# HemuManju/carla-imitation-learning

Hardware: NVIDIA B200
Metric: bc_train_frames_per_sec (higher is better)
Workload: dtype bf16

## Files before the change

### carla_imitation_learning_b200/csrc/stage.cu

```cuda
#include "bc_common.cuh"

namespace {

__device__ __forceinline__ float gray_px(uint32_t r, uint32_t g, uint32_t b) {
    const float s = (float)(299u * r + 587u * g + 114u * b);
    const float rcp = 1.0f / 255000.0f;
    const float q0 = __fmul_rn(s, rcp);
    const float rem = __fmaf_rn(-q0, 255000.0f, s);
    return __fmaf_rn(rem, rcp, q0);
}

template <int PX, typename TOUT>
__global__ void __launch_bounds__(256) stage_gray_kernel(const uint8_t* __restrict__ rgb,
                                                         TOUT* __restrict__ out, int64_t n_groups) {
    const int64_t stride = (int64_t)gridDim.x * blockDim.x;
    for (int64_t g = (int64_t)blockIdx.x * blockDim.x + threadIdx.x; g < n_groups; g += stride) {
        const uint32_t* src = reinterpret_cast<const uint32_t*>(rgb + g * (3 * PX));
        uint32_t w[3 * PX / 4];
#pragma unroll
        for (int i = 0; i < 3 * PX / 4; ++i) w[i] = __ldg(src + i);
        float v[PX];
#pragma unroll
        for (int p = 0; p < PX; ++p) {
            uint32_t c[3];
#pragma unroll
            for (int k = 0; k < 3; ++k) {
                const int byte = 3 * p + k;
                c[k] = (w[byte >> 2] >> (8 * (byte & 3))) & 0xffu;
            }
            v[p] = gray_px(c[0], c[1], c[2]);
        }
        if constexpr (sizeof(TOUT) == 4) {
            float4* dst = reinterpret_cast<float4*>(out + g * PX);
#pragma unroll
            for (int i = 0; i < PX / 4; ++i) dst[i] = make_float4(v[4 * i], v[4 * i + 1], v[4 * i + 2], v[4 * i + 3]);
        } else {
            uint32_t pk[PX / 2];
#pragma unroll
            for (int i = 0; i < PX / 2; ++i) {
                __nv_bfloat162 h = __floats2bfloat162_rn(v[2 * i], v[2 * i + 1]);
                pk[i] = *reinterpret_cast<uint32_t*>(&h);
            }
            uint4* dst = reinterpret_cast<uint4*>(out + g * PX);
#pragma unroll
            for (int i = 0; i < PX / 8; ++i) dst[i] = make_uint4(pk[4 * i], pk[4 * i + 1], pk[4 * i + 2], pk[4 * i + 3]);
        }
    }
}

constexpr int TP_NG = 21, TP_NQ = 86;

template <typename LOADER>
__device__ __forceinline__ void tp_write(LOADER&& load16, __nv_bfloat16* __restrict__ out, int64_t u) {
    const int g = (int)(u % TP_NG), q = (int)((u / TP_NG) % TP_NQ), c = (int)((u / (TP_NG * TP_NQ)) % 3);
    const int64_t plane = u / (TP_NG * TP_NQ * 3);
    const int R = 3 * q + c;
    uint32_t pk[8] = {0, 0, 0, 0, 0, 0, 0, 0};
    if (R < BC_H) load16(plane, R, 12 * g, pk);
    __nv_bfloat16* dst = out + plane * BC_TP_PLANE_ELEMS + ((int64_t)(c * 2) * TP_NQ + q) * (TP_NG * 8) + g * 8;
    *reinterpret_cast<uint4*>(dst) = make_uint4(pk[0], pk[1], pk[2], pk[3]);
    *reinterpret_cast<uint4*>(dst + TP_NQ * TP_NG * 8) = make_uint4(pk[4], pk[5], pk[6], pk[7]);
}

__device__ __forceinline__ uint32_t pack_bf16(float a, float b) {
    __nv_bfloat162 h = __floats2bfloat162_rn(a, b);
    return *reinterpret_cast<uint32_t*>(&h);
}

constexpr int TP_NU = TP_NG + 1;

__device__ __forceinline__ float gray_px_bf16_exact(uint32_t px ) {
    uint32_t acc = __dp4a(px, 0xFF72FFFFu, 0x4B000000u);
    acc = __dp4a(px, 0x00004D2Cu, acc);
    const float s = __uint_as_float(acc) - 8388608.0f;
    constexpr float r = 1.0f / 255000.0f;
    constexpr float r_lo = (float)(1.0 / 255000.0 - (double)r);
    return __fmaf_rn(s, r_lo, __fmul_rn(s, r));
}

__global__ void __launch_bounds__(256) stage_gray_tp_kernel(const uint8_t* __restrict__ rgb, __nv_bfloat16* __restrict__ out,
                                                            __nv_bfloat16* __restrict__ plain, uint32_t n_units) {
    bc::pdl_wait();
    bc::pdl_trigger();
    const uint32_t stride = gridDim.x * blockDim.x;
    for (uint32_t u = blockIdx.x * blockDim.x + threadIdx.x; u < n_units; u += stride) {
        const uint32_t t1 = u / TP_NU, g = u - t1 * TP_NU;
        const uint32_t t2 = t1 / TP_NQ, q = t1 - t2 * TP_NQ;
        const uint32_t plane = t2 / 3u, c = t2 - plane * 3u;
        const uint32_t R = 3u * q + c;
        uint32_t pk[6] = {0, 0, 0, 0, 0, 0};
        if (R < BC_H) {
            const uint32_t* src = reinterpret_cast<const uint32_t*>(rgb + ((size_t)plane * (BC_H * BC_W) + R * BC_W + 12u * g) * 3);
            uint32_t w[10];
#pragma unroll
            for (int i = 0; i < 9; ++i) w[i] = (g < TP_NG || i < 3) ? __ldg(src + i) : 0u;
            w[9] = 0u;
            float v[12];
#pragma unroll
            for (int p = 0; p < 12; ++p) {
                constexpr uint32_t sel[4] = {0x1210u, 0x2321u, 0x3432u, 0x4543u};
                const int o = (3 * p) & 3, i = (3 * p) >> 2;
                v[p] = gray_px_bf16_exact(__byte_perm(w[i], w[i + 1], sel[o]));
            }
#pragma unroll
            for (int i = 0; i < 6; ++i) pk[i] = pack_bf16(v[2 * i], v[2 * i + 1]);
            if (plain) {
                uint2* dst = reinterpret_cast<uint2*>(plain + ((size_t)plane * BC_H + R) * BC_W + 12u * g);
                dst[0] = make_uint2(pk[0], pk[1]);
                if (g < TP_NG) { dst[1] = make_uint2(pk[2], pk[3]); dst[2] = make_uint2(pk[4], pk[5]); }
            }
        }
        __nv_bfloat16* row0 = out + (size_t)plane * BC_TP_PLANE_ELEMS + ((c * 2u) * TP_NQ + q) * (TP_NG * 8);
        __nv_bfloat16* row1 = row0 + TP_NQ * TP_NG * 8;
        if (g < TP_NG) {
            *reinterpret_cast<uint4*>(row0 + g * 8) = make_uint4(pk[0], pk[1], pk[2], pk[3]);
            *reinterpret_cast<uint2*>(row1 + g * 8) = make_uint2(pk[4], pk[5]);
        }
        if (g > 0) *reinterpret_cast<uint2*>(row1 + (g - 1) * 8 + 4) = make_uint2(pk[0], pk[1]);
    }
}

template <typename TIN>
__global__ void __launch_bounds__(256) planes_to_tp_kernel(const TIN* __restrict__ in, int64_t plane_stride, __nv_bfloat16* __restrict__ out, int64_t n_units) {
    const int64_t stride = (int64_t)gridDim.x * blockDim.x;
    for (int64_t u = (int64_t)blockIdx.x * blockDim.x + threadIdx.x; u < n_units; u += stride)
        tp_write([&](int64_t plane, int R, int px0, uint32_t (&pk)[8]) {
            const TIN* src = in + plane * plane_stride + R * BC_W + px0;
            if constexpr (sizeof(TIN) == 4) {
#pragma unroll
                for (int i = 0; i < 4; ++i) {
                    const float4 f = __ldg(reinterpret_cast<const float4*>(src) + i);
                    pk[2 * i] = pack_bf16(f.x, f.y); pk[2 * i + 1] = pack_bf16(f.z, f.w);
                }
            } else {
#pragma unroll
                for (int i = 0; i < 4; ++i) {
                    const uint2 w = __ldg(reinterpret_cast<const uint2*>(src) + i);
                    pk[2 * i] = w.x; pk[2 * i + 1] = w.y;
                }
            }
        }, out, u);
}

struct AugRow { float cy, cx, br, ct, sa, mean, istd, pad; };
__device__ __forceinline__ float clamp255(float v) { return fminf(fmaxf(v, 0.f), 255.f); }
__device__ __forceinline__ float luma(float r, float g, float b) {
    return __fadd_rn(__fadd_rn(__fmul_rn(0.299f, r), __fmul_rn(0.587f, g)), __fmul_rn(0.114f, b));
}
__device__ __forceinline__ float aug_px(const uint8_t* __restrict__ px, const AugRow& t) {
    float c[3];
#pragma unroll
    for (int k = 0; k < 3; ++k) {
        float v = clamp255(__fmul_rn((float)__ldg(px + k), t.br));
        c[k] = clamp255(__fadd_rn(__fmul_rn(__fadd_rn(v, -127.5f), t.ct), 127.5f));
    }
    const float y = luma(c[0], c[1], c[2]);
#pragma unroll
    for (int k = 0; k < 3; ++k) c[k] = clamp255(__fadd_rn(y, __fmul_rn(__fadd_rn(c[k], -y), t.sa)));
    const float g = __fmul_rn(luma(c[0], c[1], c[2]), 1.0f / 255.0f);
    return __fmul_rn(__fadd_rn(g, -t.mean), t.istd);
}

__global__ void __launch_bounds__(256) stage_aug_f32_kernel(const uint8_t* __restrict__ rgb, int src_h, int src_w, const AugRow* __restrict__ table,
                                                            float* __restrict__ out, int64_t n_groups) {
    const int64_t stride = (int64_t)gridDim.x * blockDim.x;
    for (int64_t u = (int64_t)blockIdx.x * blockDim.x + threadIdx.x; u < n_groups; u += stride) {
        const int x4 = (int)(u % (BC_W / 4)), R = (int)((u / (BC_W / 4)) % BC_H);
        const int64_t plane = u / ((BC_W / 4) * BC_H);
        const AugRow t = table[plane];
        const uint8_t* src = rgb + ((plane * src_h + (int)t.cy + R) * (int64_t)src_w + (int)t.cx + 4 * x4) * 3;
        float4 v;
        v.x = aug_px(src, t); v.y = aug_px(src + 3, t); v.z = aug_px(src + 6, t); v.w = aug_px(src + 9, t);
        reinterpret_cast<float4*>(out)[u] = v;
    }
}

__global__ void __launch_bounds__(256) stage_aug_tp_kernel(const uint8_t* __restrict__ rgb, int src_h, int src_w, const AugRow* __restrict__ table,
                                                           __nv_bfloat16* __restrict__ out, int64_t n_units) {
    const int64_t stride = (int64_t)gridDim.x * blockDim.x;
    for (int64_t u = (int64_t)blockIdx.x * blockDim.x + threadIdx.x; u < n_units; u += stride) {
        const int g = (int)(u % TP_NU), q = (int)((u / TP_NU) % TP_NQ), c = (int)((u / (TP_NU * TP_NQ)) % 3);
        const int64_t plane = u / (TP_NU * TP_NQ * 3);
        const int R = 3 * q + c;
        uint32_t pk[6] = {0, 0, 0, 0, 0, 0};
        if (R < BC_H) {
            const AugRow t = table[plane];
            const uint8_t* src = rgb + ((plane * src_h + (int)t.cy + R) * (int64_t)src_w + (int)t.cx + 12 * g) * 3;
            const int npx = g < TP_NG ? 12 : 4;
            float v[12];
#pragma unroll
            for (int p = 0; p < 12; ++p) v[p] = p < npx ? aug_px(src + 3 * p, t) : 0.f;
#pragma unroll
            for (int i = 0; i < 6; ++i) pk[i] = pack_bf16(v[2 * i], v[2 * i + 1]);
        }
        __nv_bfloat16* row0 = out + plane * BC_TP_PLANE_ELEMS + ((int64_t)(c * 2) * TP_NQ + q) * (TP_NG * 8);
        __nv_bfloat16* row1 = row0 + TP_NQ * TP_NG * 8;
        if (g < TP_NG) {
            *reinterpret_cast<uint4*>(row0 + g * 8) = make_uint4(pk[0], pk[1], pk[2], pk[3]);
            *reinterpret_cast<uint2*>(row1 + g * 8) = make_uint2(pk[4], pk[5]);
        }
        if (g > 0) *reinterpret_cast<uint2*>(row1 + (g - 1) * 8 + 4) = make_uint2(pk[0], pk[1]);
    }
}

}

extern "C" int bc_stage_augment(const uint8_t* rgb, int64_t n_frames, int src_h, int src_w, const float* table, void* out, int out_dtype, void* stream) {
    BC_CHECK_ARG(rgb && table && out && n_frames >= 0, "bc_stage_augment: null pointer");
    BC_CHECK_ARG(src_h >= BC_H && src_w >= BC_W, "bc_stage_augment: source frames %dx%d are smaller than the %dx%d crop", src_h, src_w, BC_H, BC_W);
    BC_CHECK_ARG(out_dtype == BC_F32 || out_dtype == BC_BF16_TP, "bc_stage_augment: output is BC_F32 planes or BC_BF16_TP planes, got %d", out_dtype);
    BC_CHECK_ARG((uintptr_t)out % 16 == 0 && (uintptr_t)table % 16 == 0, "bc_stage_augment: out and table must be 16 B aligned");
    if (n_frames == 0) return BC_OK;
    const int64_t cap = (int64_t)bc::num_sms() * 16;
    if (out_dtype == BC_F32) {
        const int64_t groups = n_frames * BC_H * (BC_W / 4);
        const int blocks = (int)((groups + 255) / 256 < cap ? (groups + 255) / 256 : cap);
        stage_aug_f32_kernel<<<blocks, 256, 0, (cudaStream_t)stream>>>(rgb, src_h, src_w, (const AugRow*)table, (float*)out, groups);
    } else {
        const int64_t units = n_frames * 3 * TP_NQ * TP_NU;
        const int blocks = (int)((units + 255) / 256 < cap ? (units + 255) / 256 : cap);
        stage_aug_tp_kernel<<<blocks, 256, 0, (cudaStream_t)stream>>>(rgb, src_h, src_w, (const AugRow*)table, (__nv_bfloat16*)out, units);
    }
    BC_CUDA_LAUNCH_CHECK("stage_aug_kernel");
    return BC_OK;
}

extern "C" int bc_planes_to_tp(const void* planes, int in_dtype, int64_t n_planes, int64_t plane_stride, void* out_tp, void* stream) {
    BC_CHECK_ARG(planes && out_tp && n_planes >= 0, "bc_planes_to_tp: null pointer");
    BC_CHECK_ARG(in_dtype == BC_F32 || in_dtype == BC_BF16, "bc_planes_to_tp: planes are f32 or bf16, got dtype %d", in_dtype);
    const int esz = in_dtype == BC_F32 ? 4 : 2;
    BC_CHECK_ARG((uintptr_t)planes % 16 == 0 && (plane_stride * esz) % 16 == 0 && (uintptr_t)out_tp % 16 == 0, "bc_planes_to_tp: 16 B alignment");
    if (n_planes == 0) return BC_OK;
    const int64_t units = n_planes * 3 * TP_NQ * TP_NG;
    int64_t blocks = (units + 255) / 256;
    const int64_t cap = (int64_t)bc::num_sms() * 16;
    if (blocks > cap) blocks = cap;
    if (in_dtype == BC_F32)
        planes_to_tp_kernel<float><<<(int)blocks, 256, 0, (cudaStream_t)stream>>>((const float*)planes, plane_stride, (__nv_bfloat16*)out_tp, units);
    else
        planes_to_tp_kernel<__nv_bfloat16><<<(int)blocks, 256, 0, (cudaStream_t)stream>>>((const __nv_bfloat16*)planes, plane_stride, (__nv_bfloat16*)out_tp, units);
    BC_CUDA_LAUNCH_CHECK("planes_to_tp_kernel");
    return BC_OK;
}

extern "C" int bc_stage_gray_tp(const uint8_t* rgb, void* tp, void* plain_bf16, int64_t n_frames, void* stream) {
    BC_CHECK_ARG(rgb && tp && n_frames >= 0, "bc_stage_gray_tp: null pointer");
    BC_CHECK_ARG(((uintptr_t)rgb % 4 == 0) && ((uintptr_t)tp % 16 == 0) && ((uintptr_t)plain_bf16 % 8 == 0), "bc_stage_gray_tp: alignment");
    if (n_frames == 0) return BC_OK;
    const int64_t units = n_frames * 3 * TP_NQ * TP_NU;
    BC_CHECK_ARG(units < (int64_t)0x7fffffff - 0x1000000, "bc_stage_gray_tp: %lld frames in one call (the unit index is 32-bit: at most 378,000)", (long long)n_frames);
    const int64_t cap = (int64_t)bc::num_sms() * 16;
    const int blocks = (int)((units + 255) / 256 < cap ? (units + 255) / 256 : cap);
    bc::launch_pdl(stage_gray_tp_kernel, dim3(blocks), dim3(256), 0, (cudaStream_t)stream, rgb, (__nv_bfloat16*)tp, (__nv_bfloat16*)plain_bf16, (uint32_t)units);
    BC_CUDA_LAUNCH_CHECK("stage_gray_tp_kernel");
    return BC_OK;
}

extern "C" int bc_stage_gray(const uint8_t* rgb, void* gray, int64_t n_pixels, int out_dtype, void* stream) {
    BC_CHECK_ARG(rgb && gray, "bc_stage_gray: null pointer");
    BC_CHECK_ARG(n_pixels >= 0 && n_pixels % 8 == 0, "bc_stage_gray: n_pixels=%lld must be a multiple of 8", (long long)n_pixels);
    BC_CHECK_ARG(((uintptr_t)rgb % 4 == 0) && ((uintptr_t)gray % 16 == 0), "bc_stage_gray: rgb must be 4 B and gray 16 B aligned");
    BC_CHECK_ARG(out_dtype == BC_F32 || out_dtype == BC_BF16 || out_dtype == BC_BF16_TP, "bc_stage_gray: bad dtype %d", out_dtype);
    if (n_pixels == 0) return BC_OK;
    cudaStream_t s = (cudaStream_t)stream;
    const int sms = bc::num_sms();
    if (out_dtype == BC_BF16_TP) {
        BC_CHECK_ARG(n_pixels % (BC_H * BC_W) == 0, "bc_stage_gray: the TP layout is defined for whole 256x256 frames");
        const int64_t units = n_pixels / (BC_H * BC_W) * 3 * TP_NQ * TP_NU;
        BC_CHECK_ARG(units < (int64_t)0x7fffffff - 0x1000000, "bc_stage_gray: too many frames in one call for the TP layout (32-bit unit index: at most 378,000)");
        int blocks = (int)((units + 255) / 256 < (int64_t)sms * 16 ? (units + 255) / 256 : (int64_t)sms * 16);
        stage_gray_tp_kernel<<<blocks, 256, 0, s>>>(rgb, (__nv_bfloat16*)gray, nullptr, (uint32_t)units);
    } else if (out_dtype == BC_F32) {
        int64_t groups = n_pixels / 4;
        int blocks = (int)((groups + 255) / 256 < (int64_t)sms * 16 ? (groups + 255) / 256 : (int64_t)sms * 16);
        stage_gray_kernel<4, float><<<blocks, 256, 0, s>>>(rgb, (float*)gray, groups);
    } else {
        int64_t groups = n_pixels / 8;
        int blocks = (int)((groups + 255) / 256 < (int64_t)sms * 16 ? (groups + 255) / 256 : (int64_t)sms * 16);
        stage_gray_kernel<8, __nv_bfloat16><<<blocks, 256, 0, s>>>(rgb, (__nv_bfloat16*)gray, groups);
    }
    BC_CUDA_LAUNCH_CHECK("stage_gray_kernel");
    return BC_OK;
}
```

Baseline: 1.330 million.

## Restructure gray TP staging kernel to warp-per-row with cp.async pipelined loads

Result: no change. 1.335 million, median of 6 (+0.3%).

```diff
diff --git a/carla_imitation_learning_b200/csrc/stage.cu b/carla_imitation_learning_b200/csrc/stage.cu
--- a/carla_imitation_learning_b200/csrc/stage.cu
+++ b/carla_imitation_learning_b200/csrc/stage.cu
@@ -78,46 +78,109 @@
     return __fmaf_rn(s, r_lo, __fmul_rn(s, r));
 }
 
-__global__ void __launch_bounds__(256) stage_gray_tp_kernel(const uint8_t* __restrict__ rgb, __nv_bfloat16* __restrict__ out,
-                                                            __nv_bfloat16* __restrict__ plain, uint32_t n_units) {
+constexpr int ST_ROWS = BC_H + 2;
+constexpr int ST_ROW_BYTES = BC_W * 3;
+constexpr int ST_STAGES = 3;
+constexpr int ST_WARPS = 8;
+constexpr int ST_CTAS_PER_SM = 8;
+
+template <int VEC>
+__device__ __forceinline__ void cp_async(void* smem, const void* gmem) {
+    const uint32_t s = (uint32_t)__cvta_generic_to_shared(smem);
+    if constexpr (VEC == 16) asm volatile("cp.async.cg.shared.global [%0], [%1], 16;" :: "r"(s), "l"(gmem) : "memory");
+    else asm volatile("cp.async.ca.shared.global [%0], [%1], 4;" :: "r"(s), "l"(gmem) : "memory");
+}
+__device__ __forceinline__ void cp_async_commit() { asm volatile("cp.async.commit_group;" ::: "memory"); }
+template <int N>
+__device__ __forceinline__ void cp_async_wait() { asm volatile("cp.async.wait_group %0;" :: "n"(N) : "memory"); }
+
+template <int VEC>
+__global__ void __launch_bounds__(ST_WARPS * 32, ST_CTAS_PER_SM) stage_gray_tp_kernel(const uint8_t* __restrict__ rgb, __nv_bfloat16* __restrict__ out,
+                                                                                     __nv_bfloat16* __restrict__ plain, uint32_t n_rows) {
+    __shared__ __align__(16) uint8_t raw_s[ST_WARPS][ST_STAGES][ST_ROW_BYTES];
+    __shared__ __align__(16) uint8_t row_s[ST_WARPS][BC_W * 2];
+    const int warp = threadIdx.x >> 5, lane = threadIdx.x & 31;
+    const uint32_t stride = gridDim.x * ST_WARPS;
+    uint32_t t = blockIdx.x * ST_WARPS + warp;
+    auto fetch = [&](uint32_t row, int stage) {
+        if (row < n_rows) {
+            const uint32_t plane = row / ST_ROWS, R = row - plane * ST_ROWS;
+            if (R < BC_H) {
+                const uint8_t* src = rgb + ((size_t)plane * BC_H + R) * ST_ROW_BYTES;
+#pragma unroll
+                for (int j = lane; j < ST_ROW_BYTES / VEC; j += 32) cp_async<VEC>(raw_s[warp][stage] + j * VEC, src + j * VEC);
+            }
+        }
+        cp_async_commit();
+    };
+#pragma unroll
+    for (int s = 0; s < ST_STAGES - 1; ++s) fetch(t + s * stride, s);
     bc::pdl_wait();
     bc::pdl_trigger();
-    const uint32_t stride = gridDim.x * blockDim.x;
-    for (uint32_t u = blockIdx.x * blockDim.x + threadIdx.x; u < n_units; u += stride) {
-        const uint32_t t1 = u / TP_NU, g = u - t1 * TP_NU;
-        const uint32_t t2 = t1 / TP_NQ, q = t1 - t2 * TP_NQ;
-        const uint32_t plane = t2 / 3u, c = t2 - plane * 3u;
-        const uint32_t R = 3u * q + c;
-        uint32_t pk[6] = {0, 0, 0, 0, 0, 0};
+    for (int stage = 0; t < n_rows; t += stride, stage = stage == ST_STAGES - 1 ? 0 : stage + 1) {
+        fetch(t + (ST_STAGES - 1) * stride, stage == 0 ? ST_STAGES - 1 : stage - 1);
+        cp_async_wait<ST_STAGES - 1>();
+        __syncwarp();
+        const uint32_t plane = t / ST_ROWS, R = t - plane * ST_ROWS;
+        uint32_t pk[4] = {0, 0, 0, 0};
         if (R < BC_H) {
-            const uint32_t* src = reinterpret_cast<const uint32_t*>(rgb + ((size_t)plane * (BC_H * BC_W) + R * BC_W + 12u * g) * 3);
-            uint32_t w[10];
-#pragma unroll
-            for (int i = 0; i < 9; ++i) w[i] = (g < TP_NG || i < 3) ? __ldg(src + i) : 0u;
-            w[9] = 0u;
-            float v[12];
-#pragma unroll
-            for (int p = 0; p < 12; ++p) {
+            const uint2* src = reinterpret_cast<const uint2*>(raw_s[warp][stage] + 24 * lane);
+            uint32_t w[7];
+#pragma unroll
+            for (int i = 0; i < 3; ++i) { const uint2 v = src[i]; w[2 * i] = v.x; w[2 * i + 1] = v.y; }
+            w[6] = 0u;
+            float v[8];
+#pragma unroll
+            for (int p = 0; p < 8; ++p) {
                 constexpr uint32_t sel[4] = {0x1210u, 0x2321u, 0x3432u, 0x4543u};
                 const int o = (3 * p) & 3, i = (3 * p) >> 2;
                 v[p] = gray_px_bf16_exact(__byte_perm(w[i], w[i + 1], sel[o]));
             }
 #pragma unroll
-            for (int i = 0; i < 6; ++i) pk[i] = pack_bf16(v[2 * i], v[2 * i + 1]);
+            for (int i = 0; i < 4; ++i) pk[i] = pack_bf16(v[2 * i], v[2 * i + 1]);
             if (plain) {
-                uint2* dst = reinterpret_cast<uint2*>(plain + ((size_t)plane * BC_H + R) * BC_W + 12u * g);
-                dst[0] = make_uint2(pk[0], pk[1]);
-                if (g < TP_NG) { dst[1] = make_uint2(pk[2], pk[3]); dst[2] = make_uint2(pk[4], pk[5]); }
-            }
-        }
+                __nv_bfloat16* dst = plain + ((size_t)plane * BC_H + R) * BC_W + 8 * lane;
+                if (((uintptr_t)plain & 15) == 0) {
+                    *reinterpret_cast<uint4*>(dst) = make_uint4(pk[0], pk[1], pk[2], pk[3]);
+                } else {
+                    reinterpret_cast<uint2*>(dst)[0] = make_uint2(pk[0], pk[1]);
+                    reinterpret_cast<uint2*>(dst)[1] = make_uint2(pk[2], pk[3]);
+                }
+            }
+        }
+        *reinterpret_cast<uint4*>(row_s[warp] + 16 * lane) = make_uint4(pk[0], pk[1], pk[2], pk[3]);
+        __syncwarp();
+        const uint32_t q = R / 3u, c = R - 3u * q;
         __nv_bfloat16* row0 = out + (size_t)plane * BC_TP_PLANE_ELEMS + ((c * 2u) * TP_NQ + q) * (TP_NG * 8);
-        __nv_bfloat16* row1 = row0 + TP_NQ * TP_NG * 8;
-        if (g < TP_NG) {
-            *reinterpret_cast<uint4*>(row0 + g * 8) = make_uint4(pk[0], pk[1], pk[2], pk[3]);
-            *reinterpret_cast<uint2*>(row1 + g * 8) = make_uint2(pk[4], pk[5]);
-        }
-        if (g > 0) *reinterpret_cast<uint2*>(row1 + (g - 1) * 8 + 4) = make_uint2(pk[0], pk[1]);
-    }
+#pragma unroll
+        for (int j = lane; j < 2 * TP_NG; j += 32) {
+            const int h = j >= TP_NG, g = j - h * TP_NG;
+            const uint2* s = reinterpret_cast<const uint2*>(row_s[warp] + 24 * g + 16 * h);
+            const uint2 a = s[0], b = s[1];
+            *reinterpret_cast<uint4*>(row0 + h * (TP_NQ * TP_NG * 8) + g * 8) = make_uint4(a.x, a.y, b.x, b.y);
+        }
+    }
+    cp_async_wait<0>();
+}
+
+int launch_stage_gray_tp(const uint8_t* rgb, __nv_bfloat16* tp, __nv_bfloat16* plain, int64_t n_frames, cudaStream_t s, bool pdl) {
+    const uint32_t rows = (uint32_t)(n_frames * ST_ROWS);
+    auto kern = ((uintptr_t)rgb % 16 == 0) ? stage_gray_tp_kernel<16> : stage_gray_tp_kernel<4>;
+    static bc::PerDeviceOnce once_; bool& configured = once_();
+    if (!configured) {
+        for (auto k : {stage_gray_tp_kernel<16>, stage_gray_tp_kernel<4>}) {
+            const cudaError_t e = cudaFuncSetAttribute(k, cudaFuncAttributePreferredSharedMemoryCarveout, (int)cudaSharedmemCarveoutMaxShared);
+            if (e != cudaSuccess) return bc::fail(BC_ERR_DEVICE, "stage_gray_tp_kernel: carveout: %s", cudaGetErrorString(e));
+        }
+        configured = true;
+    }
+    const int64_t resident = (int64_t)bc::num_sms() * ST_CTAS_PER_SM;
+    const int64_t need = (rows + ST_WARPS - 1) / ST_WARPS;
+    const dim3 grid((unsigned)(need < resident ? need : resident)), block(ST_WARPS * 32);
+    if (pdl) bc::launch_pdl(kern, grid, block, 0, s, rgb, tp, plain, rows);
+    else kern<<<grid, block, 0, s>>>(rgb, tp, plain, rows);
+    BC_CUDA_LAUNCH_CHECK("stage_gray_tp_kernel");
+    return BC_OK;
 }
 
 template <typename TIN>
@@ -249,11 +312,7 @@
     if (n_frames == 0) return BC_OK;
     const int64_t units = n_frames * 3 * TP_NQ * TP_NU;
     BC_CHECK_ARG(units < (int64_t)0x7fffffff - 0x1000000, "bc_stage_gray_tp: %lld frames in one call (the unit index is 32-bit: at most 378,000)", (long long)n_frames);
-    const int64_t cap = (int64_t)bc::num_sms() * 16;
-    const int blocks = (int)((units + 255) / 256 < cap ? (units + 255) / 256 : cap);
-    bc::launch_pdl(stage_gray_tp_kernel, dim3(blocks), dim3(256), 0, (cudaStream_t)stream, rgb, (__nv_bfloat16*)tp, (__nv_bfloat16*)plain_bf16, (uint32_t)units);
-    BC_CUDA_LAUNCH_CHECK("stage_gray_tp_kernel");
-    return BC_OK;
+    return launch_stage_gray_tp(rgb, (__nv_bfloat16*)tp, (__nv_bfloat16*)plain_bf16, n_frames, (cudaStream_t)stream, true);
 }
 
 extern "C" int bc_stage_gray(const uint8_t* rgb, void* gray, int64_t n_pixels, int out_dtype, void* stream) {
@@ -268,8 +327,7 @@
         BC_CHECK_ARG(n_pixels % (BC_H * BC_W) == 0, "bc_stage_gray: the TP layout is defined for whole 256x256 frames");
         const int64_t units = n_pixels / (BC_H * BC_W) * 3 * TP_NQ * TP_NU;
         BC_CHECK_ARG(units < (int64_t)0x7fffffff - 0x1000000, "bc_stage_gray: too many frames in one call for the TP layout (32-bit unit index: at most 378,000)");
-        int blocks = (int)((units + 255) / 256 < (int64_t)sms * 16 ? (units + 255) / 256 : (int64_t)sms * 16);
-        stage_gray_tp_kernel<<<blocks, 256, 0, s>>>(rgb, (__nv_bfloat16*)gray, nullptr, (uint32_t)units);
+        return launch_stage_gray_tp(rgb, (__nv_bfloat16*)gray, nullptr, n_pixels / (BC_H * BC_W), s, false);
     } else if (out_dtype == BC_F32) {
         int64_t groups = n_pixels / 4;
         int blocks = (int)((groups + 255) / 256 < (int64_t)sms * 16 ? (groups + 255) / 256 : (int64_t)sms * 16);
```
